# AlvinYH/Faster-VoxelPose

Hardware: AMD Instinct MI355X
Metric: frames/sec at 5-view 80x80x20 voxel (heatmaps -> 3D joints); MPJPE vs ref (mm) in mpjpe_vs_ref_mm (higher is better)
Workload: dtype f32

## Files before the change

faster-voxelpose_amd/csrc/fvp_conv_args.h:

```cpp
#pragma once
#include <hip/hip_runtime.h>

#include <cstdint>
#include <cstdlib>

#include "fvp_asm.h"
#include "fvp_common.h"

namespace fvp {

__device__ __forceinline__ int fdiv(int x, unsigned magic) { return magic ? int(__umulhi(unsigned(x), magic)) : x; }
__device__ __forceinline__ int fdiv_nb(int x, unsigned magic) {
  return int(__umulhi(unsigned(x), magic) + (unsigned(x) & (0u - unsigned(magic == 0u))));
}
typedef fvp_i32x4 i32x4;

inline unsigned make_magic(int d) { return d <= 1 ? 0u : unsigned((1ull << 32) / unsigned(d)) + 1u; }

#ifndef FVP_CONV_BUF_DMA
#define FVP_CONV_BUF_DMA 1
#endif

struct ConvArgs {
  const float* src;
  float* dst;
  const float* res;
  const float* wts;
  const float* epi;
  const uint8_t* plane_valid;
  const float* zeros;
  int valid_div;
  int planes, cin, cinp, cout, coutp;
  int H, W;
  int OH, OW;
  int osy, osx;
  int TN, TH, TW;
  int tiles_x, tiles_y;
  int CC;
  int flags;
  int ablate;
  int dma;
  int vec;
  int ntapT;
  int tapT_w;
  unsigned m_w, m_thw, m_qpr, m_rpc, m_thp;
  int tpp, tpr;
  int wino_ni;
  int nunits, ysplit;
  unsigned m_ys, m_ty;
  unsigned long long* dbg;
  float* pool_dst;
  int wrow;
  unsigned m_tpp, m_tpr;
  const float* w2;
  const float* epi2;
  float* dst2;
  int cout2, flags2;
  int nflags;
  unsigned m_vd;
  int epi_off;
};


#if defined(HIPEMU)
#define FVP_FRESH_ARGS(a) (&(a))
typedef const ConvArgs* KArgsPtr;
#else
typedef const __attribute__((address_space(4))) ConvArgs* KArgsPtr;
__device__ __forceinline__ KArgsPtr fresh_args_ptr() {
  KArgsPtr p = (KArgsPtr)__builtin_amdgcn_kernarg_segment_ptr();
  asm volatile("" : "+s"(p));
  return p;
}
#define FVP_FRESH_ARGS(a) fresh_args_ptr()
#endif

inline bool buf_dma_range_ok(int TN, int cin, int h, int w, double weight_floats) {
  const double lim = double(0x7ffffff0u);
  return (double(TN) + 2.0) * cin * h * w * 4.0 < lim && weight_floats * 4.0 < lim;
}

inline size_t env_size(const char* name, size_t dflt) {
  const char* v = fvp::diag_env(name);
  return v ? size_t(atol(v)) : dflt;
}

int persistent_workgroups();

enum class ConvForm { Reg, TPair, Wino, K7, KSplit, Pair7, Direct, Refused };
ConvForm conv_form(const FvpConvOp& op, int planes, bool has_pool_dst, bool has_head);

bool wino_shape_ok(int h, int w, int cinp, int coutp);
int wino_plan_and_launch(const FvpConvOp& op, ConvArgs a, const float* params, int planes, hipStream_t s);
int wino_pack(const float* weight, const FvpConvOp& op, float* params, hipStream_t s);

}
```

faster-voxelpose_amd/csrc/fvp_conv_wino.hip:

```cpp
#include <hip/hip_runtime.h>

#include <algorithm>
#include <cstdio>
#include <type_traits>

#include "fvp_conv_args.h"

#ifndef FVP_WINO_ABLATE
#define FVP_WINO_ABLATE 0
#endif

namespace fvp {

typedef float f32x4 __attribute__((ext_vector_type(4)));

template <int N>
__device__ __forceinline__ void wait_vmcnt_imm() {
  static_assert(N >= 0 && N < 64, "vmcnt");
  __builtin_amdgcn_s_waitcnt(0x0f70 | (N & 15) | ((N >> 4) << 14));
}

constexpr unsigned kWinoOOB = 0x80000000u;

template <int WC, int WT, int CC, int NI, bool HAS_RES, bool RESW, int CW = 2>
__global__ void __launch_bounds__(WC * WT * 64, (WC * WT == 16 ? 4 : 2)) k_conv_wino(ConvArgs a) {
  HIP_DYNAMIC_SHARED(float, smem)
  constexpr int NWV = WC * WT;
  constexpr int NT = NWV * 64;
  static_assert(NWV == 16 || NWV == 8 || NWV == 4, "4, 8 or 16 waves");
  static_assert(CW == 1 || CW == 2, "cout blocks per wave");
  static_assert(CC == 4 || CC == 8, "chunk");
  static_assert(NI >= 1 && NI <= 4, "input DMA rounds");
  constexpr int CBW = 16 * CW * WC;
  constexpr int WCH = CC * CBW * 16;
  constexpr int WS_SZ = RESW ? 0 : WCH;
  constexpr int NW = RESW ? 0 : CC * CBW * 4 / NT;
  static_assert(RESW || (CC * CBW * 4) % NT == 0, "whole weight DMA rounds");
  constexpr int NPS = NI + NW;
  constexpr int S = CC / 4;
  constexpr int XS_SZ = NI * NT * 4;
  constexpr int BUF_SZ = XS_SZ + WS_SZ;
  constexpr bool kDiag = FVP_WINO_ABLATE != 0;
  const int t = threadIdx.x, lane = t & 63;
  const int wave = __builtin_amdgcn_readfirstlane(t >> 6);
  const int k4 = lane >> 4, l15 = lane & 15;
  const int wc = wave % WC, wt = wave / WC;
  const int W = a.W, THp = a.TH + 2, WP = W + 4;
  const int plane_sz = THp * WP;
  const int CS = a.TN * plane_sz;
  const int ablate = kDiag ? a.ablate : 0;
  const bool dma = !(ablate & 1);

  const int epi_off = 4 + 3 * BUF_SZ + (RESW ? a.cinp * CBW * 16 : 0);
  const unsigned char* const vflag = reinterpret_cast<const unsigned char*>(smem + epi_off + 3 * a.coutp);

  const int G = gridDim.x, nunits = a.nunits;
  auto next_unit = [&](int u, auto from_lds) {
    if (a.nflags > 0) {
      while (u < nunits) {
        const int pg = fdiv_nb(fdiv_nb(u, a.m_ys), a.m_ty);
        const int f = fdiv_nb(pg, a.m_vd);
        const int ok = decltype(from_lds)::value ? int(vflag[f]) : int(a.plane_valid[f]);
        if (__builtin_amdgcn_readfirstlane(ok)) break;
        u += G;
      }
    }
    return u;
  };
  using LdsFlags = std::integral_constant<bool, true>;
  using GlobalFlags = std::integral_constant<bool, false>;
  int u = next_unit(int(blockIdx.x), GlobalFlags{});
  if (u >= nunits) return;

  const int q0 = wt * 16 + l15;
  int poff;
  {
    const bool q_ok = q0 < a.TN * a.tpp;
    const int q = q_ok ? q0 : 0;
    const int tn = fdiv_nb(q, a.m_tpp), trem = q - tn * a.tpp;
    const int ty = fdiv_nb(trem, a.m_tpr), tx = trem - ty * a.tpr;
    poff = tn * plane_sz + 2 * ty * WP + 3 + 2 * tx + k4 * CS;
  }
  const int swz = (l15 >> 2) & 3;
  const int a0 = (k4 * CBW + wc * (16 * CW) + l15) * 16 + swz * 4;
  int aoff[4];
#pragma unroll
  for (int xi = 0; xi < 4; ++xi) aoff[xi] = a0 ^ (xi << 2);
  const float* const wres = smem + 4 + 3 * BUF_SZ;
  auto wchunk = [&](const float* slot, int k) { return RESW ? wres + k * WCH : slot + XS_SZ; };

  f32x4 acc[CW][16];

  const int HW = a.H * W;
  const int nchunks = a.cinp / CC;

  unsigned voff[NI];
  auto item_pos = [&](int j, int& ry, int& n, bool& inside, int& ci, int& qd) {
    const int qpr = (W >> 2) + 1;
    const int rows_per_ch = a.TN * THp;
    const int nin = CC * rows_per_ch * qpr + 1;
    int ln = lane;
    FVP_OPAQUE_V(ln);
    const int it = (wave + NWV * j) * 64 + ln;
    const int row = fdiv_nb(it, a.m_qpr);
    qd = it - row * qpr;
    ci = fdiv_nb(row, a.m_rpc);
    const int rem = row - ci * rows_per_ch;
    n = fdiv_nb(rem, a.m_thp);
    ry = rem - n * THp;
    inside = it < nin && qd > 0 && ci < CC;
  };
#pragma unroll
  for (int j = 0; j < NI; ++j) {
    int ry, n, ci, qd;
    bool inside;
    item_pos(j, ry, n, inside, ci, qd);
    voff[j] = inside ? unsigned((n * a.cin + ci) * HW + ry * W + 4 * (qd - 1)) * 4u : 0u;
    __builtin_amdgcn_sched_barrier(0);
  }
  constexpr int DCI = NT / (CBW * 4);
  const unsigned woffb = (unsigned(t / (CBW * 4)) * unsigned(a.coutp) * 16u + 4u * unsigned(t % (CBW * 4))) * 4u;
  const unsigned wdj4 = unsigned(DCI) * unsigned(a.coutp) * 64u;
  const unsigned in_step4 = unsigned(CC) * unsigned(HW) * 4u;
  const unsigned w_step4 = unsigned(CC) * unsigned(a.coutp) * 64u;
  const unsigned lds0 = FVP_LDS_BYTE_ADDRESS(smem) + 16u + unsigned(wave) * 1024u;
  i32x4 rs_in = {0, 0, 0x7ffffff0, 0x00020000}, rs_w = {0, 0, 0x7ffffff0, 0x00020000};
  auto set_base = [](i32x4& rs, const float* p) {
    const unsigned long long b = reinterpret_cast<unsigned long long>(p);
    rs[0] = __builtin_amdgcn_readfirstlane(int(unsigned(b)));
    rs[1] = __builtin_amdgcn_readfirstlane(int(unsigned(b >> 32) & 0xffffu));
  };
  int su = u, sk = 0;
  auto enter_unit = [&](int su_) {
    const KArgsPtr ka = FVP_FRESH_ARGS(a);
    const int ys = ka->ysplit, tys = ka->tiles_y;
    const int st = fdiv_nb(su_, ka->m_ys), sy = su_ - st * ys;
    const int spg = fdiv_nb(st, ka->m_ty), sty = st - spg * tys;
    const int splane0 = spg * ka->TN, sy0 = sty * ka->TH;
    const int H = ka->H, planes = ka->planes;
    set_base(rs_in, ka->src + size_t(splane0) * ka->cin * HW + sy0 * W - W);
    set_base(rs_w, ka->wts + size_t(sy) * (CBW * 16));
#pragma unroll
    for (int j = 0; j < NI; ++j) {
      int ry, n, ci, qd;
      bool inside;
      item_pos(j, ry, n, inside, ci, qd);
      const bool ok = inside && unsigned(sy0 + ry - 1) < unsigned(H) && splane0 + n < planes;
      voff[j] = (voff[j] & 0x7fffffffu) | (ok ? 0u : kWinoOOB);
      __builtin_amdgcn_sched_barrier(0);
    }
  };
  auto stage = [&](int k, int slot) {
    const unsigned la0 = lds0 + unsigned(slot) * unsigned(BUF_SZ * 4);
    const unsigned so_in = unsigned(k) * in_step4;
#pragma unroll
    for (int j = 0; j < NI; ++j) asm_buffer_load_lds16(la0 + unsigned(NWV * j) * 1024u, voff[j], rs_in, so_in);
    const unsigned so_w = unsigned(k) * w_step4;
#pragma unroll
    for (int j = 0; j < NW; ++j)
      asm_buffer_load_lds16(la0 + unsigned(XS_SZ * 4 + NWV * j * 1024), woffb, rs_w, so_w + unsigned(j) * wdj4);
  };
  enter_unit(su);
  auto stage_next = [&](int slot, auto from_lds) {
    if (su >= nunits) return false;
    stage(sk, slot);
    if (++sk == nchunks) {
      sk = 0;
      su = next_unit(su + G, from_lds);
      if (su < nunits) enter_unit(su);
    }
    return true;
  };

  float4 av[CW][4];
  float d[4][4];
  float v[4][4];
  auto fetch_a = [&](int cb, const float* wbase, int s) {
    if (kDiag && (ablate & 256)) return;
    int a0o = a0;
    if (CW == 1) FVP_OPAQUE_V(a0o);
#pragma unroll
    for (int xi = 0; xi < 4; ++xi)
      av[cb][xi] = *reinterpret_cast<const float4*>(wbase + (CW == 1 ? (a0o ^ (xi << 2)) : aoff[xi]) + (s * 4 * CBW * 16 + cb * 256));
  };
  auto fetch_d = [&](const float* base, int s, int wp) {
    const float* xs = base + poff + s * 4 * CS;
#pragma unroll
    for (int r = 0; r < 4; ++r) {
      const float* row = xs + r * wp;
      const float2 m = *reinterpret_cast<const float2*>(row + 1);
      d[r][0] = row[0];
      d[r][1] = m.x;
      d[r][2] = m.y;
      d[r][3] = row[3];
    }
  };
  auto transform = [&](float (&tr)[4][4]) {
#pragma unroll
    for (int c = 0; c < 4; ++c) {
      tr[0][c] = d[0][c] - d[2][c];
      tr[1][c] = d[1][c] + d[2][c];
      tr[2][c] = d[2][c] - d[1][c];
      tr[3][c] = d[1][c] - d[3][c];
    }
  };
  auto columns = [&](const float (&tr)[4][4]) {
#pragma unroll
    for (int xi = 0; xi < 4; ++xi) {
      v[xi][0] = tr[xi][0] - tr[xi][2];
      v[xi][1] = tr[xi][1] + tr[xi][2];
      v[xi][2] = tr[xi][2] - tr[xi][1];
      v[xi][3] = tr[xi][1] - tr[xi][3];
    }
  };
  auto mfma16 = [&](int cb, auto firstc) {
    if (kDiag && (ablate & 4)) return;
    const f32x4 z = {0.0f, 0.0f, 0.0f, 0.0f};
#pragma unroll
    for (int xi = 0; xi < 4; ++xi) {
      const float aw[4] = {av[cb][xi].x, av[cb][xi].y, av[cb][xi].z, av[cb][xi].w};
#pragma unroll
      for (int nu = 0; nu < 4; ++nu)
        acc[cb][4 * xi + nu] = __builtin_amdgcn_mfma_f32_16x16x4f32(
            aw[nu], v[xi][nu], decltype(firstc)::value ? z : acc[cb][4 * xi + nu], 0, 0, 0);
    }
  };

  if (RESW) {
    const int rounds = (a.cinp * CBW * 4) / NT;
    for (int j = 0; j < rounds; ++j)
      asm_global_load_lds16(a.wts + size_t((wave + NWV * j) * 64 + lane) * 4,
                            __builtin_amdgcn_readfirstlane(FVP_LDS_BYTE_ADDRESS(smem) +
                                                           4u * unsigned(4 + 3 * BUF_SZ + (wave + NWV * j) * 256)));
  }
  {
    float* const e = const_cast<float*>(smem) + epi_off;
    for (int i = t; i < 3 * a.coutp; i += NT) e[i] = a.epi[i];
    unsigned char* const f = const_cast<unsigned char*>(vflag);
    for (int i = t; i < a.nflags; i += NT) f[i] = a.plane_valid[i];
  }
  if (dma) {
    stage_next(0, GlobalFlags{});
    stage_next(1, GlobalFlags{});
  }
  wait_vmcnt_imm<0>();
  __syncthreads();

  int cur = 0;
  auto slot_ptr = [&](int slot) { return smem + 4 + slot * BUF_SZ; };
  fetch_a(0, wchunk(slot_ptr(0), 0), 0);
  fetch_d(slot_ptr(0), 0, WP);
  while (true) {
    auto chunk = [&](int k, auto firstc) {
      constexpr bool kFirst = decltype(firstc)::value;
      const int nxt = cur == 2 ? 0 : cur + 1;
      const int nn = nxt == 2 ? 0 : nxt + 1;
      const bool more = dma && stage_next(nn, LdsFlags{});
      const float* const cs = slot_ptr(cur);
      const float* const ns = slot_ptr(nxt);
      int wp = WP;
      FVP_OPAQUE(wp);
      if constexpr (CW == 2) {
#pragma unroll
      for (int s = 0; s < S; ++s) {
        __builtin_amdgcn_s_waitcnt(0xc07f);
        __builtin_amdgcn_sched_barrier(0);
        fetch_a(1, wchunk(cs, k), s);
        __builtin_amdgcn_sched_barrier(0);
        float tr[4][4];
        if (kDiag && (ablate & 512)) {
#pragma unroll
          for (int r = 0; r < 4; ++r)
#pragma unroll
            for (int c = 0; c < 4; ++c) v[r][c] = d[r][c];
        } else {
          transform(tr);
        }
        if (s + 1 < S) fetch_d(cs, s + 1, wp);
        __builtin_amdgcn_sched_barrier(0);
        if (!(kDiag && (ablate & 512))) columns(tr);
        if (kFirst && s == 0) mfma16(0, std::integral_constant<bool, true>{});
        else mfma16(0, std::integral_constant<bool, false>{});
        __builtin_amdgcn_sched_barrier(0);
        __builtin_amdgcn_s_waitcnt(0xc07f);
        __builtin_amdgcn_sched_barrier(0);
        if (s + 1 < S) {
          fetch_a(0, wchunk(cs, k), s + 1);
        } else {
          if (!kFirst && dma) {
            if (more) wait_vmcnt_imm<NPS>();
            else wait_vmcnt_imm<0>();
          }
          if (!(kDiag && (ablate & 128))) __builtin_amdgcn_s_barrier();
          if (k + 1 < nchunks) {
            fetch_a(0, wchunk(ns, k + 1), 0);
            fetch_d(ns, 0, wp);
          }
        }
        __builtin_amdgcn_sched_barrier(0);
        if (kFirst && s == 0) mfma16(1, std::integral_constant<bool, true>{});
        else mfma16(1, std::integral_constant<bool, false>{});
        __builtin_amdgcn_sched_barrier(0);
      }
      } else {
#pragma unroll
        for (int s = 0; s < S; ++s) {
          __builtin_amdgcn_s_waitcnt(0xc07f);
          __builtin_amdgcn_sched_barrier(0);
          {
            float tr[4][4];
            transform(tr);
            columns(tr);
          }
          __builtin_amdgcn_sched_barrier(0);
          if (kFirst && s == 0) mfma16(0, std::integral_constant<bool, true>{});
          else mfma16(0, std::integral_constant<bool, false>{});
          __builtin_amdgcn_sched_barrier(0);
          if (s + 1 < S) {
            fetch_a(0, wchunk(cs, k), s + 1);
            fetch_d(cs, s + 1, wp);
          } else {
            if (!kFirst && dma) {
              if (more) wait_vmcnt_imm<NPS>();
              else wait_vmcnt_imm<0>();
            }
            __builtin_amdgcn_s_barrier();
            if (k + 1 < nchunks) {
              fetch_a(0, wchunk(ns, k + 1), 0);
              fetch_d(ns, 0, wp);
            }
          }
          __builtin_amdgcn_sched_barrier(0);
        }
      }
      cur = nxt;
    };
    chunk(0, std::integral_constant<bool, true>{});
    for (int k = 1; k < nchunks; ++k) chunk(k, std::integral_constant<bool, false>{});

    if (!(ablate & 8)) {
      const KArgsPtr ka = FVP_FRESH_ARGS(a);
      const int ys = ka->ysplit, tys = ka->tiles_y;
      const int ut = fdiv_nb(u, ka->m_ys), uy = u - ut * ys;
      const int pg = fdiv_nb(ut, ka->m_ty), ty_i = ut - pg * tys;
      const int plane0 = pg * ka->TN, y0 = ty_i * ka->TH, co0 = uy * CBW;
      const int cout = ka->cout, coutp = ka->coutp;
      const int flags = ka->flags;
      float* const dst = ka->dst;
      const float* const res = ka->res;
      float* const pool_dst = ka->pool_dst;
      int le = lane;
      FVP_OPAQUE_V(le);
      const int k4 = le >> 4;
      const int qe = wt * 16 + (le & 15);
      const bool q_ok = qe < ka->TN * ka->tpp;
      const int qq = q_ok ? qe : 0;
      const int tn = fdiv_nb(qq, ka->m_tpp), trem = qq - tn * ka->tpp;
      const int ty = fdiv_nb(trem, ka->m_tpr), tx = trem - ty * ka->tpr;
      const bool relu = flags & FVP_EPI_RELU;
      const bool res_after = flags & FVP_EPI_RES_AFTER_RELU;
      const int plane = plane0 + tn, y = y0 + 2 * ty, x = 2 * tx;
      const bool tile_ok = q_ok && plane < ka->planes && y < ka->H;
      const unsigned ppix = unsigned((y >> 1) * (W >> 1) + tx);
      const float* const epi_s = smem + epi_off;
      const bool fast = relu && !res_after;
      unsigned HW4 = unsigned(HW) * 4u, W4 = unsigned(W) * 4u, HWq4 = unsigned(HW >> 2) * 4u;
      FVP_OPAQUE(HW4);
      FVP_OPAQUE(W4);
      FVP_OPAQUE(HWq4);
      i32x4 rs = {0, 0, 0x7ffffff0, 0x00020000};
      if (HAS_RES) set_base(rs, res + size_t(plane0) * cout * HW);
      const unsigned lco = unsigned(tn * cout + co0 + wc * (16 * CW) + 4 * k4);
      const unsigned omask = (kDiag && (ablate & 1024)) ? 0x3ffffu : 0x7fffffffu;
      const unsigned voff0 = tile_ok ? ((lco * unsigned(HW) + unsigned(y * W + x)) * 4u) & omask : kWinoOOB;
      const unsigned voffp = tile_ok ? (lco * unsigned(HW >> 2) + ppix) * 4u : kWinoOOB;
      fvp_f32x2 r0[CW][4], r1[CW][4];
      if (HAS_RES && !(kDiag && (ablate & 16))) {
        unsigned so = 0;
#pragma unroll
        for (int cb = 0; cb < CW; ++cb) {
#pragma unroll
          for (int r = 0; r < 4; ++r) {
            r0[cb][r] = asm_buffer_load_f32x2(voff0, rs, so);
            r1[cb][r] = asm_buffer_load_f32x2(voff0, rs, so + W4);
            so += HW4;
            FVP_OPAQUE(so);
          }
          so += 12u * HW4;
        }
      } else {
#pragma unroll
        for (int cb = 0; cb < CW; ++cb)
#pragma unroll
          for (int r = 0; r < 4; ++r) r0[cb][r] = r1[cb][r] = fvp_f32x2{0.f, 0.f};
      }
      float o[CW][4][2][2];
#pragma unroll
      for (int cb = 0; cb < CW; ++cb)
#pragma unroll
        for (int r = 0; r < 4; ++r) {
          float s[4][2];
#pragma unroll
          for (int xi = 0; xi < 4; ++xi) {
            const float m0 = acc[cb][4 * xi][r], m1 = acc[cb][4 * xi + 1][r], m2 = acc[cb][4 * xi + 2][r],
                        m3 = acc[cb][4 * xi + 3][r];
            s[xi][0] = (m0 + m1) + m2;
            s[xi][1] = (m1 - m2) - m3;
          }
#pragma unroll
          for (int e = 0; e < 2; ++e) {
            o[cb][r][0][e] = (s[0][e] + s[1][e]) + s[2][e];
            o[cb][r][1][e] = (s[1][e] - s[2][e]) - s[3][e];
          }
        }
      __builtin_amdgcn_sched_barrier(0);
      wait_vmcnt_imm<0>();
      __builtin_amdgcn_sched_barrier(0);
      auto finalize = [&](auto fastc) {
        constexpr bool kFast = decltype(fastc)::value;
        set_base(rs, dst + size_t(plane0) * cout * HW);
        float pm[CW][4];
        unsigned sso = 0;
#pragma unroll
        for (int cb = 0; cb < CW; ++cb) {
          const int co4 = co0 + wc * (16 * CW) + cb * 16 + 4 * k4;
          f32x4 bn[3];
#pragma unroll
          for (int i = 0; i < 3; ++i) bn[i] = *reinterpret_cast<const f32x4*>(epi_s + i * coutp + co4);
#pragma unroll
          for (int r = 0; r < 4; ++r) {
            const float b = bn[0][r], sc = bn[1][r], sh = bn[2][r];
            const float rr[2][2] = {{r0[cb][r].x, r0[cb][r].y}, {r1[cb][r].x, r1[cb][r].y}};
            float vv[2][2];
#pragma unroll
            for (int i = 0; i < 2; ++i)
#pragma unroll
              for (int e = 0; e < 2; ++e) {
                float xv = bn_affine(o[cb][r][i][e], b, sc, sh);
                if (HAS_RES && (kFast || !res_after)) xv += rr[i][e];
                if (kFast || relu) xv = fmaxf(xv, 0.0f);
                if (HAS_RES && !kFast && res_after) xv += rr[i][e];
                vv[i][e] = xv;
              }
            pm[cb][r] = fmaxf(fmaxf(vv[0][0], vv[0][1]), fmaxf(vv[1][0], vv[1][1]));
            if (kDiag && (ablate & 32) && vv[0][0] != 1.2345e-30f) { sso += HW4; continue; }
            asm_buffer_store_f32x2(fvp_f32x2{vv[0][0], vv[0][1]}, voff0, rs, sso);
            asm_buffer_store_f32x2(fvp_f32x2{vv[1][0], vv[1][1]}, voff0, rs, sso + W4);
            sso += HW4;
            FVP_OPAQUE(sso);
          }
          sso += 12u * HW4;
        }
        if (pool_dst && !(kDiag && (ablate & 32))) {
          set_base(rs, pool_dst + size_t(plane0) * cout * (HW >> 2));
#pragma unroll
          for (int cb = 0; cb < CW; ++cb)
#pragma unroll
            for (int r = 0; r < 4; ++r)
              asm_buffer_store_f32(pm[cb][r], voffp, rs, unsigned(cb * 16 + r) * HWq4);
        }
      };
      if (fast) finalize(std::integral_constant<bool, true>{});
      else finalize(std::integral_constant<bool, false>{});
    } else {
      wait_vmcnt_imm<0>();
    }
    u = next_unit(u + G, LdsFlags{});
    if (u >= nunits) break;
    fetch_a(0, wchunk(slot_ptr(cur), 0), 0);
    fetch_d(slot_ptr(cur), 0, WP);
  }
}

__global__ void __launch_bounds__(256)
k_pack_wino(const float* __restrict__ w, int cin, int cout, int cinp, int coutp, float* __restrict__ dst) {
  const int i = blockIdx.x * 256 + threadIdx.x;
  if (i >= cinp * coutp) return;
  const int co = i % coutp, ci = i / coutp;
  float g[3][3];
#pragma unroll
  for (int ky = 0; ky < 3; ++ky)
#pragma unroll
    for (int kx = 0; kx < 3; ++kx)
      g[ky][kx] = (co < cout && ci < cin) ? w[(size_t(co) * cin + ci) * 9 + ky * 3 + kx] : 0.0f;
  float gg[4][3];
#pragma unroll
  for (int kx = 0; kx < 3; ++kx) {
    const float e = g[0][kx] + g[2][kx];
    gg[0][kx] = g[0][kx];
    gg[1][kx] = 0.5f * (e + g[1][kx]);
    gg[2][kx] = 0.5f * (e - g[1][kx]);
    gg[3][kx] = g[2][kx];
  }
  float* out = dst + size_t(i) * 16;
  const int swz = (co >> 2) & 3;
#pragma unroll
  for (int xi = 0; xi < 4; ++xi) {
    const float e = gg[xi][0] + gg[xi][2];
    float* o = out + 4 * (xi ^ swz);
    o[0] = gg[xi][0];
    o[1] = 0.5f * (e + gg[xi][1]);
    o[2] = 0.5f * (e - gg[xi][1]);
    o[3] = gg[xi][2];
  }
}

static const size_t kWinoLdsBudget = env_size("FVP_WINO_LDS_KB", 152) * 1024;
static const int kWinoGeneric = int(env_size("FVP_WINO_GENERIC", 0));
constexpr int kWinoMaskedMinW = 40;
static const int kWinoWC1 = int(env_size("FVP_WINO_WC1", 0));
static const int kWinoHalf = int(env_size("FVP_WINO_HALF", 0));
static const int kWinoNoResW = int(env_size("FVP_WINO_NO_RESW", 0));
static const int kWinoAblate = int(env_size("FVP_CONV_ABLATE", 0));
#ifndef FVP_WINO_W16_DEFAULT
#define FVP_WINO_W16_DEFAULT 0
#endif

int persistent_workgroups() {
  static int n = 0;
  if (!n) {
    int dev = 0, cus = 0;
    if (hipGetDevice(&dev) != hipSuccess ||
        hipDeviceGetAttribute(&cus, hipDeviceAttributeMultiprocessorCount, dev) != hipSuccess || cus <= 0)
      cus = 256;
    n = int(env_size("FVP_WINO_WGS", size_t(cus)));
  }
  return n;
}

static bool wino_tiling(int h, int w, int cinp, int coutp, int* WC, int* WT, int* TN, int* TR, bool half = false) {
  if (h < 2 || (h & 1) || w < 8 || (w & 3) || (coutp != 32 && coutp % 64 != 0) || cinp % 4 != 0) return false;
  if ((w & (w - 1)) && w < kWinoMaskedMinW && !kWinoGeneric) return false;
  *WC = (coutp == 32 || kWinoWC1 || half) ? 1 : 2;
  *WT = (half ? 4 : 8) / *WC;
  const int tpr = w / 2, TT = 16 * *WT, rows = h / 2;
  if (tpr > TT) return false;
  if (rows * tpr >= TT) {
    *TN = 1;
    *TR = TT / tpr;
  } else {
    *TN = TT / (rows * tpr);
    *TR = rows;
  }
  return true;
}

bool wino_shape_ok(int h, int w, int cinp, int coutp) {
  int WC, WT, TN, TR;
  return wino_tiling(h, w, cinp, coutp, &WC, &WT, &TN, &TR);
}

template <int WC, int WT, int CC, int NI, bool RES, bool RESW, int CW = 2>
static int launch_wino3(const ConvArgs& a, dim3 grid, size_t lds, hipStream_t s) {
  static LdsOptIn optin;
  auto k = &k_conv_wino<WC, WT, CC, NI, RES, RESW, CW>;
  if (int e = lds_opt_in(optin, reinterpret_cast<const void*>(k), 160 * 1024)) return e;
  hipLaunchKernelGGL(k, grid, dim3(WC * WT * 64), lds, s, a);
  return launch_status();
}
template <int WC, int WT, int CC, bool RESW, int CW = 2>
static int launch_wino2(const ConvArgs& a, dim3 grid, size_t lds, hipStream_t s) {
  const bool res = a.flags & FVP_EPI_RES;
  switch (a.wino_ni) {
    case 1: return res ? launch_wino3<WC, WT, CC, 1, true, RESW, CW>(a, grid, lds, s) : launch_wino3<WC, WT, CC, 1, false, RESW, CW>(a, grid, lds, s);
    case 2: return res ? launch_wino3<WC, WT, CC, 2, true, RESW, CW>(a, grid, lds, s) : launch_wino3<WC, WT, CC, 2, false, RESW, CW>(a, grid, lds, s);
    case 3: return res ? launch_wino3<WC, WT, CC, 3, true, RESW, CW>(a, grid, lds, s) : launch_wino3<WC, WT, CC, 3, false, RESW, CW>(a, grid, lds, s);
    case 4: return res ? launch_wino3<WC, WT, CC, 4, true, RESW, CW>(a, grid, lds, s) : launch_wino3<WC, WT, CC, 4, false, RESW, CW>(a, grid, lds, s);
  }
  return FVP_ELIMIT;
}
#if FVP_DIAG
template <int WC, int WT, bool RESW>
static int launch_wino16(const ConvArgs& a, dim3 grid, size_t lds, hipStream_t s) {
  const bool res = a.flags & FVP_EPI_RES;
  if (a.wino_ni == 1)
    return res ? launch_wino3<WC, WT, 8, 1, true, RESW, 1>(a, grid, lds, s) : launch_wino3<WC, WT, 8, 1, false, RESW, 1>(a, grid, lds, s);
  if (a.wino_ni == 2)
    return res ? launch_wino3<WC, WT, 8, 2, true, RESW, 1>(a, grid, lds, s) : launch_wino3<WC, WT, 8, 2, false, RESW, 1>(a, grid, lds, s);
  return FVP_ELIMIT;
}
#endif
template <int WC, int WT>
static int launch_wino(const ConvArgs& a, dim3 grid, size_t lds, hipStream_t s, bool resw) {
  if (WC == 1 && WT == 8 && resw && a.CC == 8) return launch_wino2<1, 8, 8, true>(a, grid, lds, s);
  if (a.CC == 8) return launch_wino2<WC, WT, 8, false>(a, grid, lds, s);
  return launch_wino2<WC, WT, 4, false>(a, grid, lds, s);
}

int wino_plan_and_launch(const FvpConvOp& op, ConvArgs a, const float* params, int planes, hipStream_t s) {
  int WC, WT, TN, TR;
  if (conv_form(op, planes, a.pool_dst != nullptr, a.w2 != nullptr) != ConvForm::Wino) return FVP_EINVAL;
  if (!wino_tiling(op.h, op.w, op.cinp, op.coutp, &WC, &WT, &TN, &TR, kWinoHalf == 1)) return FVP_EINVAL;
  if (kWinoHalf == 0) {
    const long units = long(ceil_div(op.h / 2, TR)) * ceil_div(planes, TN) * (op.coutp / (32 * WC));
    int wc, wt, tn, tr;
    if (units < persistent_workgroups() && wino_tiling(op.h, op.w, op.cinp, op.coutp, &wc, &wt, &tn, &tr, true)) {
      WC = wc; WT = wt; TN = tn; TR = tr;
    }
  }
#if FVP_DIAG
  static const int kW16 = int(env_size("FVP_WINO_W16", FVP_WINO_W16_DEFAULT));
#else
  constexpr int kW16 = 0;
#endif
  const bool w16 = kW16 && WC * WT == 8 && op.cinp % 8 == 0;
  static const int kQuarter = int(env_size("FVP_WINO_QUARTER", 1));
  bool quarter = false;
  if (kQuarter && !w16 && WC * WT == 4 && op.cinp % 4 == 0) {
    const long units_half = long(ceil_div(op.h / 2, TR)) * ceil_div(planes, TN) * (op.coutp / 32);
    quarter = units_half * (kQuarter == 2 ? 1 : 2) < persistent_workgroups();
  }
  const int CW = (w16 || quarter) ? 1 : 2;
  if (w16) WC *= 2;
  a.ablate = kWinoAblate;
  a.wts = params + op.wino_off;
  a.TN = TN;
  a.TH = 2 * TR;
  a.TW = op.w;
  a.tiles_x = 1;
  a.tiles_y = ceil_div(op.h / 2, TR);
  a.tpp = TR * (op.w / 2);
  a.m_tpp = make_magic(a.tpp);
  a.tpr = op.w / 2;
  a.m_tpr = make_magic(a.tpr);
  a.vec = a.dma = 1;
  a.zeros = params;
  const int CBW = 16 * CW * WC;
  const size_t resw_bytes = size_t(op.cinp) * CBW * 64;
  const size_t budget = WC * WT == 4 ? std::min<size_t>(kWinoLdsBudget, 78 * 1024) : kWinoLdsBudget;
  const size_t epi_bytes = size_t(3) * op.coutp * 4;
  a.nflags = (a.plane_valid && TN == 1) ? ceil_div(planes, a.valid_div) : 0;
  a.m_vd = make_magic(a.valid_div);
  const size_t flag_bytes = size_t(a.nflags + 15) & ~size_t(15);
  bool resw = CBW == 32 && WT == 8 && op.coutp == 32 && op.cinp % 8 == 0 && resw_bytes <= 64 * 1024 && !kWinoNoResW;
  auto slot_bytes = [&](int cc, int* ni, bool rw) {
    const size_t quads = size_t(cc) * TN * (a.TH + 2) * (op.w / 4 + 1) + 1;
    const size_t per_round = size_t(WC) * WT * 64;
    *ni = int((quads + per_round - 1) / per_round);
    return size_t(*ni) * per_round * 16 + (rw ? 0 : size_t(cc) * CBW * 64);
  };
  const size_t fixed = 64 + epi_bytes + flag_bytes;
  int CC = op.cinp % 8 == 0 ? 8 : 4, ni = 0;
  size_t slot = slot_bytes(CC, &ni, resw);
  if (resw && (3 * slot + resw_bytes + fixed > budget || ni > 4)) {
    resw = false;
    slot = slot_bytes(CC, &ni, false);
  }
  if (CC == 8 && !resw && (3 * slot + fixed > budget || ni > 4)) {
    CC = 4;
    slot = slot_bytes(CC, &ni, false);
  }
  if (3 * slot + (resw ? resw_bytes : 0) + fixed > budget || ni > 4) return FVP_ELIMIT;
  a.CC = CC;
  a.wino_ni = ni;
  if (!buf_dma_range_ok(TN, op.cin, op.h, op.w, double(op.cinp) * op.coutp * 16)) return FVP_ELIMIT;
  if ((double(TN) + 1.0) * op.cout * op.h * op.w * 4.0 >= 2147483648.0) return FVP_ELIMIT;
  a.m_qpr = make_magic(op.w / 4 + 1);
  a.m_rpc = make_magic(TN * (a.TH + 2));
  a.m_thp = make_magic(a.TH + 2);
  const size_t lds = 16 + 3 * slot + (resw ? resw_bytes : 0) + epi_bytes + flag_bytes;
  a.ysplit = op.coutp / CBW;
  a.nunits = a.tiles_y * ceil_div(planes, TN) * a.ysplit;
  a.m_ys = make_magic(a.ysplit);
  a.m_ty = make_magic(a.tiles_y);
  static const int kBalanced = int(env_size("FVP_WINO_BALANCED", 0));
  const int slots = persistent_workgroups() * (WC * WT == 4 ? 2 : 1);
  dim3 grid(kBalanced ? ceil_div(a.nunits, ceil_div(a.nunits, slots)) : std::min(a.nunits, slots), 1, 1);
  ProfScope ps(a.nunits < slots ? FVP_K_CONV_WINO_SMALL : FVP_K_CONV_WINO, s, 2.0 * op.cin * op.cout * 9.0 * op.h * op.w * planes, 1,
               prof_level() >= 2);
#if FVP_DIAG
  if (w16) {
    if (CC != 8 || ni > 2) return FVP_ELIMIT;
    if (CBW == 32) return resw ? launch_wino16<2, 8, true>(a, grid, lds, s) : launch_wino16<2, 8, false>(a, grid, lds, s);
    return launch_wino16<4, 4, false>(a, grid, lds, s);
  }
#endif
  if (quarter) return a.CC == 8 ? launch_wino2<1, 4, 8, false, 1>(a, grid, lds, s) : launch_wino2<1, 4, 4, false, 1>(a, grid, lds, s);
  if (WC * WT == 4) return launch_wino<1, 4>(a, grid, lds, s, false);
  return WC == 1 ? launch_wino<1, 8>(a, grid, lds, s, resw) : launch_wino<2, 4>(a, grid, lds, s, false);
}

int wino_pack(const float* weight, const FvpConvOp& op, float* params, hipStream_t s) {
  hipLaunchKernelGGL(k_pack_wino, dim3(ceil_div(op.cinp * op.coutp, 256)), dim3(256), 0, s, weight, op.cin, op.cout,
                     op.cinp, op.coutp, params + op.wino_off);
  return launch_status();
}

}
```

Before: 3016.

## Add shared-column Winograd conv kernel using DPP row-neighbour exchange

Adds a Winograd F(2x2,3x3) conv kernel variant (k_conv_wsc) in which lanes holding adjacent tiles share overlapping input columns through DPP row shifts instead of each reading all four columns from LDS. The tile-to-lane mapping is permuted (SH==2) so that neighbours sit in adjacent lanes, and the epilogue undoes the permutation. The intent is to cut LDS read traffic in the input transform, at the cost of extra cross-lane ops and a more complex lane mapping. A new shcols argument and a shared-instance predicate control which configurations use it.

```diff
diff --git a/faster-voxelpose_amd/csrc/fvp_conv_args.h b/faster-voxelpose_amd/csrc/fvp_conv_args.h
--- a/faster-voxelpose_amd/csrc/fvp_conv_args.h
+++ b/faster-voxelpose_amd/csrc/fvp_conv_args.h
@@ -59,6 +59,7 @@
   int nflags;
   unsigned m_vd;
   int epi_off;
+  int shcols;
 };
 
 
@@ -74,6 +75,19 @@
 }
 #define FVP_FRESH_ARGS(a) fresh_args_ptr()
 #endif
+
+template <int SHIFT, bool LEFT>
+__device__ __forceinline__ float dpp_row_neighbour(float x) {
+  static_assert(SHIFT >= 1 && SHIFT <= 15, "row shift");
+#if defined(HIPEMU)
+  const int lane = hipemu::cur->lane, src = LEFT ? lane - SHIFT : lane + SHIFT;
+  const bool inside = src >= 0 && (src >> 4) == (lane >> 4);
+  const float r = hipemu_shfl_from(x, inside ? src : lane);
+  return inside ? r : 0.0f;
+#else
+  return __int_as_float(__builtin_amdgcn_update_dpp(0, __float_as_int(x), (LEFT ? 0x110 : 0x100) + SHIFT, 0xf, 0xf, true));
+#endif
+}
 
 inline bool buf_dma_range_ok(int TN, int cin, int h, int w, double weight_floats) {
   const double lim = double(0x7ffffff0u);
diff --git a/faster-voxelpose_amd/csrc/fvp_conv_wino.hip b/faster-voxelpose_amd/csrc/fvp_conv_wino.hip
--- a/faster-voxelpose_amd/csrc/fvp_conv_wino.hip
+++ b/faster-voxelpose_amd/csrc/fvp_conv_wino.hip
@@ -22,454 +22,29 @@
 
 constexpr unsigned kWinoOOB = 0x80000000u;
 
+constexpr bool wino_shared_instance(int WC, int WT, int CC, int NI) {
+  return WC == 2 ? (WT == 4 && NI == (CC == 8 ? 2 : 1)) : WT == 4 ? (CC == 4 && NI == 2) : (WT == 8 && NI == (CC == 8 ? 3 : 2));
+}
+
+template <int WC, int WT, int CC, int NI, bool HAS_RES, bool RESW, int SH>
+__global__ void k_conv_wsc(ConvArgs a);
+
 template <int WC, int WT, int CC, int NI, bool HAS_RES, bool RESW, int CW = 2>
 __global__ void __launch_bounds__(WC * WT * 64, (WC * WT == 16 ? 4 : 2)) k_conv_wino(ConvArgs a) {
-  HIP_DYNAMIC_SHARED(float, smem)
-  constexpr int NWV = WC * WT;
-  constexpr int NT = NWV * 64;
-  static_assert(NWV == 16 || NWV == 8 || NWV == 4, "4, 8 or 16 waves");
-  static_assert(CW == 1 || CW == 2, "cout blocks per wave");
-  static_assert(CC == 4 || CC == 8, "chunk");
-  static_assert(NI >= 1 && NI <= 4, "input DMA rounds");
-  constexpr int CBW = 16 * CW * WC;
-  constexpr int WCH = CC * CBW * 16;
-  constexpr int WS_SZ = RESW ? 0 : WCH;
-  constexpr int NW = RESW ? 0 : CC * CBW * 4 / NT;
-  static_assert(RESW || (CC * CBW * 4) % NT == 0, "whole weight DMA rounds");
-  constexpr int NPS = NI + NW;
-  constexpr int S = CC / 4;
-  constexpr int XS_SZ = NI * NT * 4;
-  constexpr int BUF_SZ = XS_SZ + WS_SZ;
-  constexpr bool kDiag = FVP_WINO_ABLATE != 0;
-  const int t = threadIdx.x, lane = t & 63;
-  const int wave = __builtin_amdgcn_readfirstlane(t >> 6);
-  const int k4 = lane >> 4, l15 = lane & 15;
-  const int wc = wave % WC, wt = wave / WC;
-  const int W = a.W, THp = a.TH + 2, WP = W + 4;
-  const int plane_sz = THp * WP;
-  const int CS = a.TN * plane_sz;
-  const int ablate = kDiag ? a.ablate : 0;
-  const bool dma = !(ablate & 1);
-
-  const int epi_off = 4 + 3 * BUF_SZ + (RESW ? a.cinp * CBW * 16 : 0);
-  const unsigned char* const vflag = reinterpret_cast<const unsigned char*>(smem + epi_off + 3 * a.coutp);
-
-  const int G = gridDim.x, nunits = a.nunits;
-  auto next_unit = [&](int u, auto from_lds) {
-    if (a.nflags > 0) {
-      while (u < nunits) {
-        const int pg = fdiv_nb(fdiv_nb(u, a.m_ys), a.m_ty);
-        const int f = fdiv_nb(pg, a.m_vd);
-        const int ok = decltype(from_lds)::value ? int(vflag[f]) : int(a.plane_valid[f]);
-        if (__builtin_amdgcn_readfirstlane(ok)) break;
-        u += G;
-      }
-    }
-    return u;
-  };
-  using LdsFlags = std::integral_constant<bool, true>;
-  using GlobalFlags = std::integral_constant<bool, false>;
-  int u = next_unit(int(blockIdx.x), GlobalFlags{});
-  if (u >= nunits) return;
-
-  const int q0 = wt * 16 + l15;
-  int poff;
-  {
-    const bool q_ok = q0 < a.TN * a.tpp;
-    const int q = q_ok ? q0 : 0;
-    const int tn = fdiv_nb(q, a.m_tpp), trem = q - tn * a.tpp;
-    const int ty = fdiv_nb(trem, a.m_tpr), tx = trem - ty * a.tpr;
-    poff = tn * plane_sz + 2 * ty * WP + 3 + 2 * tx + k4 * CS;
-  }
-  const int swz = (l15 >> 2) & 3;
-  const int a0 = (k4 * CBW + wc * (16 * CW) + l15) * 16 + swz * 4;
-  int aoff[4];
-#pragma unroll
-  for (int xi = 0; xi < 4; ++xi) aoff[xi] = a0 ^ (xi << 2);
-  const float* const wres = smem + 4 + 3 * BUF_SZ;
-  auto wchunk = [&](const float* slot, int k) { return RESW ? wres + k * WCH : slot + XS_SZ; };
-
-  f32x4 acc[CW][16];
-
-  const int HW = a.H * W;
-  const int nchunks = a.cinp / CC;
-
-  unsigned voff[NI];
-  auto item_pos = [&](int j, int& ry, int& n, bool& inside, int& ci, int& qd) {
-    const int qpr = (W >> 2) + 1;
-    const int rows_per_ch = a.TN * THp;
-    const int nin = CC * rows_per_ch * qpr + 1;
-    int ln = lane;
-    FVP_OPAQUE_V(ln);
-    const int it = (wave + NWV * j) * 64 + ln;
-    const int row = fdiv_nb(it, a.m_qpr);
-    qd = it - row * qpr;
-    ci = fdiv_nb(row, a.m_rpc);
-    const int rem = row - ci * rows_per_ch;
-    n = fdiv_nb(rem, a.m_thp);
-    ry = rem - n * THp;
-    inside = it < nin && qd > 0 && ci < CC;
-  };
-#pragma unroll
-  for (int j = 0; j < NI; ++j) {
-    int ry, n, ci, qd;
-    bool inside;
-    item_pos(j, ry, n, inside, ci, qd);
-    voff[j] = inside ? unsigned((n * a.cin + ci) * HW + ry * W + 4 * (qd - 1)) * 4u : 0u;
-    __builtin_amdgcn_sched_barrier(0);
-  }
-  constexpr int DCI = NT / (CBW * 4);
-  const unsigned woffb = (unsigned(t / (CBW * 4)) * unsigned(a.coutp) * 16u + 4u * unsigned(t % (CBW * 4))) * 4u;
-  const unsigned wdj4 = unsigned(DCI) * unsigned(a.coutp) * 64u;
-  const unsigned in_step4 = unsigned(CC) * unsigned(HW) * 4u;
-  const unsigned w_step4 = unsigned(CC) * unsigned(a.coutp) * 64u;
-  const unsigned lds0 = FVP_LDS_BYTE_ADDRESS(smem) + 16u + unsigned(wave) * 1024u;
-  i32x4 rs_in = {0, 0, 0x7ffffff0, 0x00020000}, rs_w = {0, 0, 0x7ffffff0, 0x00020000};
-  auto set_base = [](i32x4& rs, const float* p) {
-    const unsigned long long b = reinterpret_cast<unsigned long long>(p);
-    rs[0] = __builtin_amdgcn_readfirstlane(int(unsigned(b)));
-    rs[1] = __builtin_amdgcn_readfirstlane(int(unsigned(b >> 32) & 0xffffu));
-  };
-  int su = u, sk = 0;
-  auto enter_unit = [&](int su_) {
-    const KArgsPtr ka = FVP_FRESH_ARGS(a);
-    const int ys = ka->ysplit, tys = ka->tiles_y;
-    const int st = fdiv_nb(su_, ka->m_ys), sy = su_ - st * ys;
-    const int spg = fdiv_nb(st, ka->m_ty), sty = st - spg * tys;
-    const int splane0 = spg * ka->TN, sy0 = sty * ka->TH;
-    const int H = ka->H, planes = ka->planes;
-    set_base(rs_in, ka->src + size_t(splane0) * ka->cin * HW + sy0 * W - W);
-    set_base(rs_w, ka->wts + size_t(sy) * (CBW * 16));
-#pragma unroll
-    for (int j = 0; j < NI; ++j) {
-      int ry, n, ci, qd;
-      bool inside;
-      item_pos(j, ry, n, inside, ci, qd);
-      const bool ok = inside && unsigned(sy0 + ry - 1) < unsigned(H) && splane0 + n < planes;
-      voff[j] = (voff[j] & 0x7fffffffu) | (ok ? 0u : kWinoOOB);
-      __builtin_amdgcn_sched_barrier(0);
-    }
-  };
-  auto stage = [&](int k, int slot) {
-    const unsigned la0 = lds0 + unsigned(slot) * unsigned(BUF_SZ * 4);
-    const unsigned so_in = unsigned(k) * in_step4;
-#pragma unroll
-    for (int j = 0; j < NI; ++j) asm_buffer_load_lds16(la0 + unsigned(NWV * j) * 1024u, voff[j], rs_in, so_in);
-    const unsigned so_w = unsigned(k) * w_step4;
-#pragma unroll
-    for (int j = 0; j < NW; ++j)
-      asm_buffer_load_lds16(la0 + unsigned(XS_SZ * 4 + NWV * j * 1024), woffb, rs_w, so_w + unsigned(j) * wdj4);
-  };
-  enter_unit(su);
-  auto stage_next = [&](int slot, auto from_lds) {
-    if (su >= nunits) return false;
-    stage(sk, slot);
-    if (++sk == nchunks) {
-      sk = 0;
-      su = next_unit(su + G, from_lds);
-      if (su < nunits) enter_unit(su);
-    }
-    return true;
-  };
-
-  float4 av[CW][4];
-  float d[4][4];
-  float v[4][4];
-  auto fetch_a = [&](int cb, const float* wbase, int s) {
-    if (kDiag && (ablate & 256)) return;
-    int a0o = a0;
-    if (CW == 1) FVP_OPAQUE_V(a0o);
-#pragma unroll
-    for (int xi = 0; xi < 4; ++xi)
-      av[cb][xi] = *reinterpret_cast<const float4*>(wbase + (CW == 1 ? (a0o ^ (xi << 2)) : aoff[xi]) + (s * 4 * CBW * 16 + cb * 256));
-  };
-  auto fetch_d = [&](const float* base, int s, int wp) {
-    const float* xs = base + poff + s * 4 * CS;
-#pragma unroll
-    for (int r = 0; r < 4; ++r) {
-      const float* row = xs + r * wp;
-      const float2 m = *reinterpret_cast<const float2*>(row + 1);
-      d[r][0] = row[0];
-      d[r][1] = m.x;
-      d[r][2] = m.y;
-      d[r][3] = row[3];
-    }
-  };
-  auto transform = [&](float (&tr)[4][4]) {
-#pragma unroll
-    for (int c = 0; c < 4; ++c) {
-      tr[0][c] = d[0][c] - d[2][c];
-      tr[1][c] = d[1][c] + d[2][c];
-      tr[2][c] = d[2][c] - d[1][c];
-      tr[3][c] = d[1][c] - d[3][c];
-    }
-  };
-  auto columns = [&](const float (&tr)[4][4]) {
-#pragma unroll
-    for (int xi = 0; xi < 4; ++xi) {
-      v[xi][0] = tr[xi][0] - tr[xi][2];
-      v[xi][1] = tr[xi][1] + tr[xi][2];
-      v[xi][2] = tr[xi][2] - tr[xi][1];
-      v[xi][3] = tr[xi][1] - tr[xi][3];
-    }
-  };
-  auto mfma16 = [&](int cb, auto firstc) {
-    if (kDiag && (ablate & 4)) return;
-    const f32x4 z = {0.0f, 0.0f, 0.0f, 0.0f};
-#pragma unroll
-    for (int xi = 0; xi < 4; ++xi) {
-      const float aw[4] = {av[cb][xi].x, av[cb][xi].y, av[cb][xi].z, av[cb][xi].w};
-#pragma unroll
-      for (int nu = 0; nu < 4; ++nu)
-        acc[cb][4 * xi + nu] = __builtin_amdgcn_mfma_f32_16x16x4f32(
-            aw[nu], v[xi][nu], decltype(firstc)::value ? z : acc[cb][4 * xi + nu], 0, 0, 0);
-    }
-  };
-
-  if (RESW) {
-    const int rounds = (a.cinp * CBW * 4) / NT;
-    for (int j = 0; j < rounds; ++j)
-      asm_global_load_lds16(a.wts + size_t((wave + NWV * j) * 64 + lane) * 4,
-                            __builtin_amdgcn_readfirstlane(FVP_LDS_BYTE_ADDRESS(smem) +
-                                                           4u * unsigned(4 + 3 * BUF_SZ + (wave + NWV * j) * 256)));
-  }
-  {
-    float* const e = const_cast<float*>(smem) + epi_off;
-    for (int i = t; i < 3 * a.coutp; i += NT) e[i] = a.epi[i];
-    unsigned char* const f = const_cast<unsigned char*>(vflag);
-    for (int i = t; i < a.nflags; i += NT) f[i] = a.plane_valid[i];
-  }
-  if (dma) {
-    stage_next(0, GlobalFlags{});
-    stage_next(1, GlobalFlags{});
-  }
-  wait_vmcnt_imm<0>();
-  __syncthreads();
-
-  int cur = 0;
-  auto slot_ptr = [&](int slot) { return smem + 4 + slot * BUF_SZ; };
-  fetch_a(0, wchunk(slot_ptr(0), 0), 0);
-  fetch_d(slot_ptr(0), 0, WP);
-  while (true) {
-    auto chunk = [&](int k, auto firstc) {
-      constexpr bool kFirst = decltype(firstc)::value;
-      const int nxt = cur == 2 ? 0 : cur + 1;
-      const int nn = nxt == 2 ? 0 : nxt + 1;
-      const bool more = dma && stage_next(nn, LdsFlags{});
-      const float* const cs = slot_ptr(cur);
-      const float* const ns = slot_ptr(nxt);
-      int wp = WP;
-      FVP_OPAQUE(wp);
-      if constexpr (CW == 2) {
-#pragma unroll
-      for (int s = 0; s < S; ++s) {
-        __builtin_amdgcn_s_waitcnt(0xc07f);
-        __builtin_amdgcn_sched_barrier(0);
-        fetch_a(1, wchunk(cs, k), s);
-        __builtin_amdgcn_sched_barrier(0);
-        float tr[4][4];
-        if (kDiag && (ablate & 512)) {
-#pragma unroll
-          for (int r = 0; r < 4; ++r)
-#pragma unroll
-            for (int c = 0; c < 4; ++c) v[r][c] = d[r][c];
-        } else {
-          transform(tr);
-        }
-        if (s + 1 < S) fetch_d(cs, s + 1, wp);
-        __builtin_amdgcn_sched_barrier(0);
-        if (!(kDiag && (ablate & 512))) columns(tr);
-        if (kFirst && s == 0) mfma16(0, std::integral_constant<bool, true>{});
-        else mfma16(0, std::integral_constant<bool, false>{});
-        __builtin_amdgcn_sched_barrier(0);
-        __builtin_amdgcn_s_waitcnt(0xc07f);
-        __builtin_amdgcn_sched_barrier(0);
-        if (s + 1 < S) {
-          fetch_a(0, wchunk(cs, k), s + 1);
-        } else {
-          if (!kFirst && dma) {
-            if (more) wait_vmcnt_imm<NPS>();
-            else wait_vmcnt_imm<0>();
-          }
-          if (!(kDiag && (ablate & 128))) __builtin_amdgcn_s_barrier();
-          if (k + 1 < nchunks) {
-            fetch_a(0, wchunk(ns, k + 1), 0);
-            fetch_d(ns, 0, wp);
-          }
-        }
-        __builtin_amdgcn_sched_barrier(0);
-        if (kFirst && s == 0) mfma16(1, std::integral_constant<bool, true>{});
-        else mfma16(1, std::integral_constant<bool, false>{});
-        __builtin_amdgcn_sched_barrier(0);
-      }
-      } else {
-#pragma unroll
-        for (int s = 0; s < S; ++s) {
-          __builtin_amdgcn_s_waitcnt(0xc07f);
-          __builtin_amdgcn_sched_barrier(0);
-          {
-            float tr[4][4];
-            transform(tr);
-            columns(tr);
-          }
-          __builtin_amdgcn_sched_barrier(0);
-          if (kFirst && s == 0) mfma16(0, std::integral_constant<bool, true>{});
-          else mfma16(0, std::integral_constant<bool, false>{});
-          __builtin_amdgcn_sched_barrier(0);
-          if (s + 1 < S) {
-            fetch_a(0, wchunk(cs, k), s + 1);
-            fetch_d(cs, s + 1, wp);
-          } else {
-            if (!kFirst && dma) {
-              if (more) wait_vmcnt_imm<NPS>();
-              else wait_vmcnt_imm<0>();
-            }
-            __builtin_amdgcn_s_barrier();
-            if (k + 1 < nchunks) {
-              fetch_a(0, wchunk(ns, k + 1), 0);
-              fetch_d(ns, 0, wp);
-            }
-          }
-          __builtin_amdgcn_sched_barrier(0);
-        }
-      }
-      cur = nxt;
-    };
-    chunk(0, std::integral_constant<bool, true>{});
-    for (int k = 1; k < nchunks; ++k) chunk(k, std::integral_constant<bool, false>{});
-
-    if (!(ablate & 8)) {
-      const KArgsPtr ka = FVP_FRESH_ARGS(a);
-      const int ys = ka->ysplit, tys = ka->tiles_y;
-      const int ut = fdiv_nb(u, ka->m_ys), uy = u - ut * ys;
-      const int pg = fdiv_nb(ut, ka->m_ty), ty_i = ut - pg * tys;
-      const int plane0 = pg * ka->TN, y0 = ty_i * ka->TH, co0 = uy * CBW;
-      const int cout = ka->cout, coutp = ka->coutp;
-      const int flags = ka->flags;
-      float* const dst = ka->dst;
-      const float* const res = ka->res;
-      float* const pool_dst = ka->pool_dst;
-      int le = lane;
-      FVP_OPAQUE_V(le);
-      const int k4 = le >> 4;
-      const int qe = wt * 16 + (le & 15);
-      const bool q_ok = qe < ka->TN * ka->tpp;
-      const int qq = q_ok ? qe : 0;
-      const int tn = fdiv_nb(qq, ka->m_tpp), trem = qq - tn * ka->tpp;
-      const int ty = fdiv_nb(trem, ka->m_tpr), tx = trem - ty * ka->tpr;
-      const bool relu = flags & FVP_EPI_RELU;
-      const bool res_after = flags & FVP_EPI_RES_AFTER_RELU;
-      const int plane = plane0 + tn, y = y0 + 2 * ty, x = 2 * tx;
-      const bool tile_ok = q_ok && plane < ka->planes && y < ka->H;
-      const unsigned ppix = unsigned((y >> 1) * (W >> 1) + tx);
-      const float* const epi_s = smem + epi_off;
-      const bool fast = relu && !res_after;
-      unsigned HW4 = unsigned(HW) * 4u, W4 = unsigned(W) * 4u, HWq4 = unsigned(HW >> 2) * 4u;
-      FVP_OPAQUE(HW4);
-      FVP_OPAQUE(W4);
-      FVP_OPAQUE(HWq4);
-      i32x4 rs = {0, 0, 0x7ffffff0, 0x00020000};
-      if (HAS_RES) set_base(rs, res + size_t(plane0) * cout * HW);
-      const unsigned lco = unsigned(tn * cout + co0 + wc * (16 * CW) + 4 * k4);
-      const unsigned omask = (kDiag && (ablate & 1024)) ? 0x3ffffu : 0x7fffffffu;
-      const unsigned voff0 = tile_ok ? ((lco * unsigned(HW) + unsigned(y * W + x)) * 4u) & omask : kWinoOOB;
-      const unsigned voffp = tile_ok ? (lco * unsigned(HW >> 2) + ppix) * 4u : kWinoOOB;
-      fvp_f32x2 r0[CW][4], r1[CW][4];
-      if (HAS_RES && !(kDiag && (ablate & 16))) {
-        unsigned so = 0;
-#pragma unroll
-        for (int cb = 0; cb < CW; ++cb) {
-#pragma unroll
-          for (int r = 0; r < 4; ++r) {
-            r0[cb][r] = asm_buffer_load_f32x2(voff0, rs, so);
-            r1[cb][r] = asm_buffer_load_f32x2(voff0, rs, so + W4);
-            so += HW4;
-            FVP_OPAQUE(so);
-          }
-          so += 12u * HW4;
-        }
-      } else {
-#pragma unroll
-        for (int cb = 0; cb < CW; ++cb)
-#pragma unroll
-          for (int r = 0; r < 4; ++r) r0[cb][r] = r1[cb][r] = fvp_f32x2{0.f, 0.f};
-      }
-      float o[CW][4][2][2];
-#pragma unroll
-      for (int cb = 0; cb < CW; ++cb)
-#pragma unroll
-        for (int r = 0; r < 4; ++r) {
-          float s[4][2];
-#pragma unroll
-          for (int xi = 0; xi < 4; ++xi) {
-            const float m0 = acc[cb][4 * xi][r], m1 = acc[cb][4 * xi + 1][r], m2 = acc[cb][4 * xi + 2][r],
-                        m3 = acc[cb][4 * xi + 3][r];
-            s[xi][0] = (m0 + m1) + m2;
-            s[xi][1] = (m1 - m2) - m3;
-          }
-#pragma unroll
-          for (int e = 0; e < 2; ++e) {
-            o[cb][r][0][e] = (s[0][e] + s[1][e]) + s[2][e];
-            o[cb][r][1][e] = (s[1][e] - s[2][e]) - s[3][e];
-          }
-        }
-      __builtin_amdgcn_sched_barrier(0);
-      wait_vmcnt_imm<0>();
-      __builtin_amdgcn_sched_barrier(0);
-      auto finalize = [&](auto fastc) {
-        constexpr bool kFast = decltype(fastc)::value;
-        set_base(rs, dst + size_t(plane0) * cout * HW);
-        float pm[CW][4];
-        unsigned sso = 0;
-#pragma unroll
-        for (int cb = 0; cb < CW; ++cb) {
-          const int co4 = co0 + wc * (16 * CW) + cb * 16 + 4 * k4;
-          f32x4 bn[3];
-#pragma unroll
-          for (int i = 0; i < 3; ++i) bn[i] = *reinterpret_cast<const f32x4*>(epi_s + i * coutp + co4);
-#pragma unroll
-          for (int r = 0; r < 4; ++r) {
-            const float b = bn[0][r], sc = bn[1][r], sh = bn[2][r];
-            const float rr[2][2] = {{r0[cb][r].x, r0[cb][r].y}, {r1[cb][r].x, r1[cb][r].y}};
-            float vv[2][2];
-#pragma unroll
-            for (int i = 0; i < 2; ++i)
-#pragma unroll
-              for (int e = 0; e < 2; ++e) {
-                float xv = bn_affine(o[cb][r][i][e], b, sc, sh);
-                if (HAS_RES && (kFast || !res_after)) xv += rr[i][e];
-                if (kFast || relu) xv = fmaxf(xv, 0.0f);
-                if (HAS_RES && !kFast && res_after) xv += rr[i][e];
-                vv[i][e] = xv;
-              }
-            pm[cb][r] = fmaxf(fmaxf(vv[0][0], vv[0][1]), fmaxf(vv[1][0], vv[1][1]));
-            if (kDiag && (ablate & 32) && vv[0][0] != 1.2345e-30f) { sso += HW4; continue; }
-            asm_buffer_store_f32x2(fvp_f32x2{vv[0][0], vv[0][1]}, voff0, rs, sso);
-            asm_buffer_store_f32x2(fvp_f32x2{vv[1][0], vv[1][1]}, voff0, rs, sso + W4);
-            sso += HW4;
-            FVP_OPAQUE(sso);
-          }
-          sso += 12u * HW4;
-        }
-        if (pool_dst && !(kDiag && (ablate & 32))) {
-          set_base(rs, pool_dst + size_t(plane0) * cout * (HW >> 2));
-#pragma unroll
-          for (int cb = 0; cb < CW; ++cb)
-#pragma unroll
-            for (int r = 0; r < 4; ++r)
-              asm_buffer_store_f32(pm[cb][r], voffp, rs, unsigned(cb * 16 + r) * HWq4);
-        }
-      };
-      if (fast) finalize(std::integral_constant<bool, true>{});
-      else finalize(std::integral_constant<bool, false>{});
-    } else {
-      wait_vmcnt_imm<0>();
-    }
-    u = next_unit(u + G, LdsFlags{});
-    if (u >= nunits) break;
-    fetch_a(0, wchunk(slot_ptr(cur), 0), 0);
-    fetch_d(slot_ptr(cur), 0, WP);
-  }
+#if defined(HIPEMU)
+  if constexpr (CW == 2 && wino_shared_instance(WC, WT, CC, NI)) {
+    if (a.shcols == 1) return k_conv_wsc<WC, WT, CC, NI, HAS_RES, RESW, 1>(a);
+    if (a.shcols == 2) return k_conv_wsc<WC, WT, CC, NI, HAS_RES, RESW, 2>(a);
+  }
+#endif
+  constexpr int SH = 0;
+#include "fvp_conv_wino_body.h"
+}
+
+template <int WC, int WT, int CC, int NI, bool HAS_RES, bool RESW, int SH>
+__global__ void __launch_bounds__(WC * WT * 64, 2) k_conv_wsc(ConvArgs a) {
+  constexpr int CW = 2;
+#include "fvp_conv_wino_body.h"
 }
 
 __global__ void __launch_bounds__(256)
@@ -550,8 +125,29 @@
   return wino_tiling(h, w, cinp, coutp, &WC, &WT, &TN, &TR);
 }
 
+#if defined(HIPEMU)
+template <int SH> void wino_shared_columns_form() {}
+#endif
+template <int WC, int WT, int CC, int NI, bool RES, bool RESW, int SH>
+static int launch_wsc(const ConvArgs& a, dim3 grid, size_t lds, hipStream_t s) {
+  static LdsOptIn optin;
+  auto k = &k_conv_wsc<WC, WT, CC, NI, RES, RESW, SH>;
+  if (int e = lds_opt_in(optin, reinterpret_cast<const void*>(k), 160 * 1024)) return e;
+  hipLaunchKernelGGL(k, grid, dim3(WC * WT * 64), lds, s, a);
+  return launch_status();
+}
 template <int WC, int WT, int CC, int NI, bool RES, bool RESW, int CW = 2>
 static int launch_wino3(const ConvArgs& a, dim3 grid, size_t lds, hipStream_t s) {
+#if !defined(HIPEMU)
+  if constexpr (CW == 2 && wino_shared_instance(WC, WT, CC, NI)) {
+    if (a.shcols == 1) return launch_wsc<WC, WT, CC, NI, RES, RESW, 1>(a, grid, lds, s);
+    if (a.shcols == 2) return launch_wsc<WC, WT, CC, NI, RES, RESW, 2>(a, grid, lds, s);
+  }
+  if (a.shcols) return FVP_EINVAL;
+#else
+  if (a.shcols == 1) hipemu::log_launch(reinterpret_cast<const void*>(&wino_shared_columns_form<1>));
+  if (a.shcols == 2) hipemu::log_launch(reinterpret_cast<const void*>(&wino_shared_columns_form<2>));
+#endif
   static LdsOptIn optin;
   auto k = &k_conv_wino<WC, WT, CC, NI, RES, RESW, CW>;
   if (int e = lds_opt_in(optin, reinterpret_cast<const void*>(k), 160 * 1024)) return e;
@@ -612,6 +208,7 @@
   }
   const int CW = (w16 || quarter) ? 1 : 2;
   if (w16) WC *= 2;
+  static const int kSharedCols = int(env_size("FVP_WINO_SHARED_COLS", 3));
   a.ablate = kWinoAblate;
   a.wts = params + op.wino_off;
   a.TN = TN;
@@ -653,6 +250,11 @@
   if (3 * slot + (resw ? resw_bytes : 0) + fixed > budget || ni > 4) return FVP_ELIMIT;
   a.CC = CC;
   a.wino_ni = ni;
+  a.shcols = 0;
+  if (CW == 2 && !w16 && TN == 1 && wino_shared_instance(WC, WT, CC, ni)) {
+    if (op.w == 32 && (kSharedCols & 1)) a.shcols = 1;
+    if (op.w == 16 && TR % 2 == 0 && (kSharedCols & 2)) a.shcols = 2;
+  }
   if (!buf_dma_range_ok(TN, op.cin, op.h, op.w, double(op.cinp) * op.coutp * 16)) return FVP_ELIMIT;
   if ((double(TN) + 1.0) * op.cout * op.h * op.w * 4.0 >= 2147483648.0) return FVP_ELIMIT;
   a.m_qpr = make_magic(op.w / 4 + 1);
diff --git a/faster-voxelpose_amd/csrc/fvp_conv_wino_body.h b/faster-voxelpose_amd/csrc/fvp_conv_wino_body.h
--- /dev/null
+++ b/faster-voxelpose_amd/csrc/fvp_conv_wino_body.h
@@ -0,0 +1,456 @@
+  static_assert(SH == 0 || ((SH == 1 || SH == 2) && CW == 2), "shared columns: two-block waves");
+  HIP_DYNAMIC_SHARED(float, smem)
+  constexpr int NWV = WC * WT;
+  constexpr int NT = NWV * 64;
+  static_assert(NWV == 16 || NWV == 8 || NWV == 4, "4, 8 or 16 waves");
+  static_assert(CW == 1 || CW == 2, "cout blocks per wave");
+  static_assert(CC == 4 || CC == 8, "chunk");
+  static_assert(NI >= 1 && NI <= 4, "input DMA rounds");
+  constexpr int CBW = 16 * CW * WC;
+  constexpr int WCH = CC * CBW * 16;
+  constexpr int WS_SZ = RESW ? 0 : WCH;
+  constexpr int NW = RESW ? 0 : CC * CBW * 4 / NT;
+  static_assert(RESW || (CC * CBW * 4) % NT == 0, "whole weight DMA rounds");
+  constexpr int NPS = NI + NW;
+  constexpr int S = CC / 4;
+  constexpr int XS_SZ = NI * NT * 4;
+  constexpr int BUF_SZ = XS_SZ + WS_SZ;
+  constexpr bool kDiag = FVP_WINO_ABLATE != 0;
+  const int t = threadIdx.x, lane = t & 63;
+  const int wave = __builtin_amdgcn_readfirstlane(t >> 6);
+  const int k4 = lane >> 4, l15 = lane & 15;
+  const int wc = wave % WC, wt = wave / WC;
+  const int W = a.W, THp = a.TH + 2, WP = W + 4;
+  const int plane_sz = THp * WP;
+  const int CS = a.TN * plane_sz;
+  const int ablate = kDiag ? a.ablate : 0;
+  const bool dma = !(ablate & 1);
+
+  const int epi_off = 4 + 3 * BUF_SZ + (RESW ? a.cinp * CBW * 16 : 0);
+  const unsigned char* const vflag = reinterpret_cast<const unsigned char*>(smem + epi_off + 3 * a.coutp);
+
+  const int G = gridDim.x, nunits = a.nunits;
+  auto next_unit = [&](int u, auto from_lds) {
+    if (a.nflags > 0) {
+      while (u < nunits) {
+        const int pg = fdiv_nb(fdiv_nb(u, a.m_ys), a.m_ty);
+        const int f = fdiv_nb(pg, a.m_vd);
+        const int ok = decltype(from_lds)::value ? int(vflag[f]) : int(a.plane_valid[f]);
+        if (__builtin_amdgcn_readfirstlane(ok)) break;
+        u += G;
+      }
+    }
+    return u;
+  };
+  using LdsFlags = std::integral_constant<bool, true>;
+  using GlobalFlags = std::integral_constant<bool, false>;
+  int u = next_unit(int(blockIdx.x), GlobalFlags{});
+  if (u >= nunits) return;
+
+  const int q0 = wt * 16 + (SH == 2 ? ((l15 & 1) << 3) | (l15 >> 1) : l15);
+  int poff;
+  {
+    const bool q_ok = q0 < a.TN * a.tpp;
+    const int q = q_ok ? q0 : 0;
+    const int tn = fdiv_nb(q, a.m_tpp), trem = q - tn * a.tpp;
+    const int ty = fdiv_nb(trem, a.m_tpr), tx = trem - ty * a.tpr;
+    poff = tn * plane_sz + 2 * ty * WP + 3 + 2 * tx + k4 * CS;
+  }
+  const int swz = (l15 >> 2) & 3;
+  const int a0 = (k4 * CBW + wc * (16 * CW) + l15) * 16 + swz * 4;
+  int aoff[4];
+#pragma unroll
+  for (int xi = 0; xi < 4; ++xi) aoff[xi] = a0 ^ (xi << 2);
+  const float* const wres = smem + 4 + 3 * BUF_SZ;
+  auto wchunk = [&](const float* slot, int k) { return RESW ? wres + k * WCH : slot + XS_SZ; };
+
+  f32x4 acc[CW][16];
+
+  const int HW = a.H * W;
+  const int nchunks = a.cinp / CC;
+
+  unsigned voff[NI];
+  auto item_pos = [&](int j, int& ry, int& n, bool& inside, int& ci, int& qd) {
+    const int qpr = (W >> 2) + 1;
+    const int rows_per_ch = a.TN * THp;
+    const int nin = CC * rows_per_ch * qpr + 1;
+    int ln = lane;
+    FVP_OPAQUE_V(ln);
+    const int it = (wave + NWV * j) * 64 + ln;
+    const int row = fdiv_nb(it, a.m_qpr);
+    qd = it - row * qpr;
+    ci = fdiv_nb(row, a.m_rpc);
+    const int rem = row - ci * rows_per_ch;
+    n = fdiv_nb(rem, a.m_thp);
+    ry = rem - n * THp;
+    inside = it < nin && qd > 0 && ci < CC;
+  };
+#pragma unroll
+  for (int j = 0; j < NI; ++j) {
+    int ry, n, ci, qd;
+    bool inside;
+    item_pos(j, ry, n, inside, ci, qd);
+    voff[j] = inside ? unsigned((n * a.cin + ci) * HW + ry * W + 4 * (qd - 1)) * 4u : 0u;
+    __builtin_amdgcn_sched_barrier(0);
+  }
+  constexpr int DCI = NT / (CBW * 4);
+  const unsigned woffb = (unsigned(t / (CBW * 4)) * unsigned(a.coutp) * 16u + 4u * unsigned(t % (CBW * 4))) * 4u;
+  const unsigned wdj4 = unsigned(DCI) * unsigned(a.coutp) * 64u;
+  const unsigned in_step4 = unsigned(CC) * unsigned(HW) * 4u;
+  const unsigned w_step4 = unsigned(CC) * unsigned(a.coutp) * 64u;
+  const unsigned lds0 = FVP_LDS_BYTE_ADDRESS(smem) + 16u + unsigned(wave) * 1024u;
+  i32x4 rs_in = {0, 0, 0x7ffffff0, 0x00020000}, rs_w = {0, 0, 0x7ffffff0, 0x00020000};
+  auto set_base = [](i32x4& rs, const float* p) {
+    const unsigned long long b = reinterpret_cast<unsigned long long>(p);
+    rs[0] = __builtin_amdgcn_readfirstlane(int(unsigned(b)));
+    rs[1] = __builtin_amdgcn_readfirstlane(int(unsigned(b >> 32) & 0xffffu));
+  };
+  int su = u, sk = 0;
+  auto enter_unit = [&](int su_) {
+    const KArgsPtr ka = FVP_FRESH_ARGS(a);
+    const int ys = ka->ysplit, tys = ka->tiles_y;
+    const int st = fdiv_nb(su_, ka->m_ys), sy = su_ - st * ys;
+    const int spg = fdiv_nb(st, ka->m_ty), sty = st - spg * tys;
+    const int splane0 = spg * ka->TN, sy0 = sty * ka->TH;
+    const int H = ka->H, planes = ka->planes;
+    set_base(rs_in, ka->src + size_t(splane0) * ka->cin * HW + sy0 * W - W);
+    set_base(rs_w, ka->wts + size_t(sy) * (CBW * 16));
+#pragma unroll
+    for (int j = 0; j < NI; ++j) {
+      int ry, n, ci, qd;
+      bool inside;
+      item_pos(j, ry, n, inside, ci, qd);
+      const bool ok = inside && unsigned(sy0 + ry - 1) < unsigned(H) && splane0 + n < planes;
+      voff[j] = (voff[j] & 0x7fffffffu) | (ok ? 0u : kWinoOOB);
+      __builtin_amdgcn_sched_barrier(0);
+    }
+  };
+  auto stage = [&](int k, int slot) {
+    const unsigned la0 = lds0 + unsigned(slot) * unsigned(BUF_SZ * 4);
+    const unsigned so_in = unsigned(k) * in_step4;
+#pragma unroll
+    for (int j = 0; j < NI; ++j) asm_buffer_load_lds16(la0 + unsigned(NWV * j) * 1024u, voff[j], rs_in, so_in);
+    const unsigned so_w = unsigned(k) * w_step4;
+#pragma unroll
+    for (int j = 0; j < NW; ++j)
+      asm_buffer_load_lds16(la0 + unsigned(XS_SZ * 4 + NWV * j * 1024), woffb, rs_w, so_w + unsigned(j) * wdj4);
+  };
+  enter_unit(su);
+  auto stage_next = [&](int slot, auto from_lds) {
+    if (su >= nunits) return false;
+    stage(sk, slot);
+    if (++sk == nchunks) {
+      sk = 0;
+      su = next_unit(su + G, from_lds);
+      if (su < nunits) enter_unit(su);
+    }
+    return true;
+  };
+
+  float4 av[CW][4];
+  float d[4][4];
+  float v[4][4];
+  auto fetch_a = [&](int cb, const float* wbase, int s) {
+    if (kDiag && (ablate & 256)) return;
+    int a0o = a0;
+    if (CW == 1) FVP_OPAQUE_V(a0o);
+#pragma unroll
+    for (int xi = 0; xi < 4; ++xi)
+      av[cb][xi] = *reinterpret_cast<const float4*>(wbase + (CW == 1 ? (a0o ^ (xi << 2)) : aoff[xi]) + (s * 4 * CBW * 16 + cb * 256));
+  };
+  auto fetch_d = [&](const float* base, int s, int wp) {
+    const float* xs = base + poff + s * 4 * CS;
+#pragma unroll
+    for (int r = 0; r < 4; ++r) {
+      const float* row = xs + r * wp;
+      const float2 m = *reinterpret_cast<const float2*>(row + 1);
+      if (SH == 0) d[r][0] = row[0];
+      d[r][1] = m.x;
+      d[r][2] = m.y;
+      if (SH == 0) d[r][3] = row[3];
+    }
+  };
+  auto transform = [&](float (&tr)[4][4]) {
+#pragma unroll
+    for (int c = (SH ? 1 : 0); c < (SH ? 3 : 4); ++c) {
+      tr[0][c] = d[0][c] - d[2][c];
+      tr[1][c] = d[1][c] + d[2][c];
+      tr[2][c] = d[2][c] - d[1][c];
+      tr[3][c] = d[1][c] - d[3][c];
+    }
+  };
+  auto columns = [&](const float (&tr)[4][4]) {
+#pragma unroll
+    for (int xi = 0; xi < 4; ++xi) {
+      if constexpr (SH == 0) {
+        v[xi][0] = tr[xi][0] - tr[xi][2];
+      } else {
+        v[xi][0] = dpp_row_neighbour<SH, true>(tr[xi][2]) - tr[xi][2];
+      }
+      v[xi][1] = tr[xi][1] + tr[xi][2];
+      v[xi][2] = tr[xi][2] - tr[xi][1];
+      if constexpr (SH == 0) {
+        v[xi][3] = tr[xi][1] - tr[xi][3];
+      } else {
+        v[xi][3] = tr[xi][1] - dpp_row_neighbour<SH, false>(tr[xi][1]);
+      }
+    }
+  };
+  auto mfma16 = [&](int cb, auto firstc) {
+    if (kDiag && (ablate & 4)) return;
+    const f32x4 z = {0.0f, 0.0f, 0.0f, 0.0f};
+#pragma unroll
+    for (int xi = 0; xi < 4; ++xi) {
+      const float aw[4] = {av[cb][xi].x, av[cb][xi].y, av[cb][xi].z, av[cb][xi].w};
+#pragma unroll
+      for (int nu = 0; nu < 4; ++nu)
+        acc[cb][4 * xi + nu] = __builtin_amdgcn_mfma_f32_16x16x4f32(
+            aw[nu], v[xi][nu], decltype(firstc)::value ? z : acc[cb][4 * xi + nu], 0, 0, 0);
+    }
+  };
+
+  if (RESW) {
+    const int rounds = (a.cinp * CBW * 4) / NT;
+    for (int j = 0; j < rounds; ++j)
+      asm_global_load_lds16(a.wts + size_t((wave + NWV * j) * 64 + lane) * 4,
+                            __builtin_amdgcn_readfirstlane(FVP_LDS_BYTE_ADDRESS(smem) +
+                                                           4u * unsigned(4 + 3 * BUF_SZ + (wave + NWV * j) * 256)));
+  }
+  {
+    float* const e = const_cast<float*>(smem) + epi_off;
+    for (int i = t; i < 3 * a.coutp; i += NT) e[i] = a.epi[i];
+    unsigned char* const f = const_cast<unsigned char*>(vflag);
+    for (int i = t; i < a.nflags; i += NT) f[i] = a.plane_valid[i];
+  }
+  if (dma) {
+    stage_next(0, GlobalFlags{});
+    stage_next(1, GlobalFlags{});
+  }
+  wait_vmcnt_imm<0>();
+  __syncthreads();
+
+  int cur = 0;
+  auto slot_ptr = [&](int slot) { return smem + 4 + slot * BUF_SZ; };
+  fetch_a(0, wchunk(slot_ptr(0), 0), 0);
+  fetch_d(slot_ptr(0), 0, WP);
+  while (true) {
+    auto chunk = [&](int k, auto firstc) {
+      constexpr bool kFirst = decltype(firstc)::value;
+      const int nxt = cur == 2 ? 0 : cur + 1;
+      const int nn = nxt == 2 ? 0 : nxt + 1;
+      const bool more = dma && stage_next(nn, LdsFlags{});
+      const float* const cs = slot_ptr(cur);
+      const float* const ns = slot_ptr(nxt);
+      int wp = WP;
+      FVP_OPAQUE(wp);
+      if constexpr (CW == 2) {
+#pragma unroll
+      for (int s = 0; s < S; ++s) {
+        __builtin_amdgcn_s_waitcnt(0xc07f);
+        __builtin_amdgcn_sched_barrier(0);
+        fetch_a(1, wchunk(cs, k), s);
+        __builtin_amdgcn_sched_barrier(0);
+        float tr[4][4];
+        if (kDiag && (ablate & 512)) {
+#pragma unroll
+          for (int r = 0; r < 4; ++r)
+#pragma unroll
+            for (int c = 0; c < 4; ++c) v[r][c] = d[r][(SH && (c == 0 || c == 3)) ? 1 : c];
+        } else {
+          transform(tr);
+        }
+        if (s + 1 < S) fetch_d(cs, s + 1, wp);
+        __builtin_amdgcn_sched_barrier(0);
+        if (!(kDiag && (ablate & 512))) columns(tr);
+        if (kFirst && s == 0) mfma16(0, std::integral_constant<bool, true>{});
+        else mfma16(0, std::integral_constant<bool, false>{});
+        __builtin_amdgcn_sched_barrier(0);
+        __builtin_amdgcn_s_waitcnt(0xc07f);
+        __builtin_amdgcn_sched_barrier(0);
+        if (s + 1 < S) {
+          fetch_a(0, wchunk(cs, k), s + 1);
+        } else {
+          if (!kFirst && dma) {
+            if (more) wait_vmcnt_imm<NPS>();
+            else wait_vmcnt_imm<0>();
+          }
+          if (!(kDiag && (ablate & 128))) __builtin_amdgcn_s_barrier();
+          if (k + 1 < nchunks) {
+            fetch_a(0, wchunk(ns, k + 1), 0);
+            fetch_d(ns, 0, wp);
+          }
+        }
+        __builtin_amdgcn_sched_barrier(0);
+        if (kFirst && s == 0) mfma16(1, std::integral_constant<bool, true>{});
+        else mfma16(1, std::integral_constant<bool, false>{});
+        __builtin_amdgcn_sched_barrier(0);
+      }
+      } else {
+#pragma unroll
+        for (int s = 0; s < S; ++s) {
+          __builtin_amdgcn_s_waitcnt(0xc07f);
+          __builtin_amdgcn_sched_barrier(0);
+          {
+            float tr[4][4];
+            transform(tr);
+            columns(tr);
+          }
+          __builtin_amdgcn_sched_barrier(0);
+          if (kFirst && s == 0) mfma16(0, std::integral_constant<bool, true>{});
+          else mfma16(0, std::integral_constant<bool, false>{});
+          __builtin_amdgcn_sched_barrier(0);
+          if (s + 1 < S) {
+            fetch_a(0, wchunk(cs, k), s + 1);
+            fetch_d(cs, s + 1, wp);
+          } else {
+            if (!kFirst && dma) {
+              if (more) wait_vmcnt_imm<NPS>();
+              else wait_vmcnt_imm<0>();
+            }
+            __builtin_amdgcn_s_barrier();
+            if (k + 1 < nchunks) {
+              fetch_a(0, wchunk(ns, k + 1), 0);
+              fetch_d(ns, 0, wp);
+            }
+          }
+          __builtin_amdgcn_sched_barrier(0);
+        }
+      }
+      cur = nxt;
+    };
+    chunk(0, std::integral_constant<bool, true>{});
+    for (int k = 1; k < nchunks; ++k) chunk(k, std::integral_constant<bool, false>{});
+
+    if (!(ablate & 8)) {
+      const KArgsPtr ka = FVP_FRESH_ARGS(a);
+      const int ys = ka->ysplit, tys = ka->tiles_y;
+      const int ut = fdiv_nb(u, ka->m_ys), uy = u - ut * ys;
+      const int pg = fdiv_nb(ut, ka->m_ty), ty_i = ut - pg * tys;
+      const int plane0 = pg * ka->TN, y0 = ty_i * ka->TH, co0 = uy * CBW;
+      const int cout = ka->cout, coutp = ka->coutp;
+      const int flags = ka->flags;
+      float* const dst = ka->dst;
+      const float* const res = ka->res;
+      float* const pool_dst = ka->pool_dst;
+      int le = lane;
+      FVP_OPAQUE_V(le);
+      const int k4 = le >> 4;
+      const int le15 = le & 15;
+      const int qe = wt * 16 + (SH == 2 ? ((le15 & 1) << 3) | (le15 >> 1) : le15);
+      const bool q_ok = qe < ka->TN * ka->tpp;
+      const int qq = q_ok ? qe : 0;
+      const int tn = fdiv_nb(qq, ka->m_tpp), trem = qq - tn * ka->tpp;
+      const int ty = fdiv_nb(trem, ka->m_tpr), tx = trem - ty * ka->tpr;
+      const bool relu = flags & FVP_EPI_RELU;
+      const bool res_after = flags & FVP_EPI_RES_AFTER_RELU;
+      const int plane = plane0 + tn, y = y0 + 2 * ty, x = 2 * tx;
+      const bool tile_ok = q_ok && plane < ka->planes && y < ka->H;
+      const unsigned ppix = unsigned((y >> 1) * (W >> 1) + tx);
+      const float* const epi_s = smem + epi_off;
+      const bool fast = relu && !res_after;
+      unsigned HW4 = unsigned(HW) * 4u, W4 = unsigned(W) * 4u, HWq4 = unsigned(HW >> 2) * 4u;
+      FVP_OPAQUE(HW4);
+      FVP_OPAQUE(W4);
+      FVP_OPAQUE(HWq4);
+      i32x4 rs = {0, 0, 0x7ffffff0, 0x00020000};
+      if (HAS_RES) set_base(rs, res + size_t(plane0) * cout * HW);
+      const unsigned lco = unsigned(tn * cout + co0 + wc * (16 * CW) + 4 * k4);
+      const unsigned omask = (kDiag && (ablate & 1024)) ? 0x3ffffu : 0x7fffffffu;
+      const unsigned voff0 = tile_ok ? ((lco * unsigned(HW) + unsigned(y * W + x)) * 4u) & omask : kWinoOOB;
+      const unsigned voffp = tile_ok ? (lco * unsigned(HW >> 2) + ppix) * 4u : kWinoOOB;
+      fvp_f32x2 r0[CW][4], r1[CW][4];
+      if (HAS_RES && !(kDiag && (ablate & 16))) {
+        unsigned so = 0;
+#pragma unroll
+        for (int cb = 0; cb < CW; ++cb) {
+#pragma unroll
+          for (int r = 0; r < 4; ++r) {
+            r0[cb][r] = asm_buffer_load_f32x2(voff0, rs, so);
+            r1[cb][r] = asm_buffer_load_f32x2(voff0, rs, so + W4);
+            so += HW4;
+            FVP_OPAQUE(so);
+          }
+          so += 12u * HW4;
+        }
+      } else {
+#pragma unroll
+        for (int cb = 0; cb < CW; ++cb)
+#pragma unroll
+          for (int r = 0; r < 4; ++r) r0[cb][r] = r1[cb][r] = fvp_f32x2{0.f, 0.f};
+      }
+      float o[CW][4][2][2];
+#pragma unroll
+      for (int cb = 0; cb < CW; ++cb)
+#pragma unroll
+        for (int r = 0; r < 4; ++r) {
+          float s[4][2];
+#pragma unroll
+          for (int xi = 0; xi < 4; ++xi) {
+            const float m0 = acc[cb][4 * xi][r], m1 = acc[cb][4 * xi + 1][r], m2 = acc[cb][4 * xi + 2][r],
+                        m3 = acc[cb][4 * xi + 3][r];
+            s[xi][0] = (m0 + m1) + m2;
+            s[xi][1] = (m1 - m2) - m3;
+          }
+#pragma unroll
+          for (int e = 0; e < 2; ++e) {
+            o[cb][r][0][e] = (s[0][e] + s[1][e]) + s[2][e];
+            o[cb][r][1][e] = (s[1][e] - s[2][e]) - s[3][e];
+          }
+        }
+      __builtin_amdgcn_sched_barrier(0);
+      wait_vmcnt_imm<0>();
+      __builtin_amdgcn_sched_barrier(0);
+      auto finalize = [&](auto fastc) {
+        constexpr bool kFast = decltype(fastc)::value;
+        set_base(rs, dst + size_t(plane0) * cout * HW);
+        float pm[CW][4];
+        unsigned sso = 0;
+#pragma unroll
+        for (int cb = 0; cb < CW; ++cb) {
+          const int co4 = co0 + wc * (16 * CW) + cb * 16 + 4 * k4;
+          f32x4 bn[3];
+#pragma unroll
+          for (int i = 0; i < 3; ++i) bn[i] = *reinterpret_cast<const f32x4*>(epi_s + i * coutp + co4);
+#pragma unroll
+          for (int r = 0; r < 4; ++r) {
+            const float b = bn[0][r], sc = bn[1][r], sh = bn[2][r];
+            const float rr[2][2] = {{r0[cb][r].x, r0[cb][r].y}, {r1[cb][r].x, r1[cb][r].y}};
+            float vv[2][2];
+#pragma unroll
+            for (int i = 0; i < 2; ++i)
+#pragma unroll
+              for (int e = 0; e < 2; ++e) {
+                float xv = bn_affine(o[cb][r][i][e], b, sc, sh);
+                if (HAS_RES && (kFast || !res_after)) xv += rr[i][e];
+                if (kFast || relu) xv = fmaxf(xv, 0.0f);
+                if (HAS_RES && !kFast && res_after) xv += rr[i][e];
+                vv[i][e] = xv;
+              }
+            pm[cb][r] = fmaxf(fmaxf(vv[0][0], vv[0][1]), fmaxf(vv[1][0], vv[1][1]));
+            if (kDiag && (ablate & 32) && vv[0][0] != 1.2345e-30f) { sso += HW4; continue; }
+            asm_buffer_store_f32x2(fvp_f32x2{vv[0][0], vv[0][1]}, voff0, rs, sso);
+            asm_buffer_store_f32x2(fvp_f32x2{vv[1][0], vv[1][1]}, voff0, rs, sso + W4);
+            sso += HW4;
+            FVP_OPAQUE(sso);
+          }
+          sso += 12u * HW4;
+        }
+        if (pool_dst && !(kDiag && (ablate & 32))) {
+          set_base(rs, pool_dst + size_t(plane0) * cout * (HW >> 2));
+#pragma unroll
+          for (int cb = 0; cb < CW; ++cb)
+#pragma unroll
+            for (int r = 0; r < 4; ++r)
+              asm_buffer_store_f32(pm[cb][r], voffp, rs, unsigned(cb * 16 + r) * HWq4);
+        }
+      };
+      if (fast) finalize(std::integral_constant<bool, true>{});
+      else finalize(std::integral_constant<bool, false>{});
+    } else {
+      wait_vmcnt_imm<0>();
+    }
+    u = next_unit(u + G, LdsFlags{});
+    if (u >= nunits) break;
+    fetch_a(0, wchunk(slot_ptr(cur), 0), 0);
+    fetch_d(slot_ptr(cur), 0, WP);
+  }
```

Measured after the change: 3058 (median of 6 runs). 1.4% higher.
